# OthmanB/TAMCMC-C

Measured on AMD Instinct MI355X. Metric: MCMC samples/sec (whole node), 1e5 nu-bins x 100 params x 20 tempered chains, higher is better.
Workload: dtype f64

## Files before the change

include/tamcmc_sampler.h:

```cpp
#ifndef TAMCMC_SAMPLER_H
#define TAMCMC_SAMPLER_H

#include <stdint.h>

#include "tamcmc_hip.h"

#ifdef __cplusplus
extern "C" {
#endif

typedef struct tamcmc_sampler tamcmc_sampler;

typedef struct tamcmc_sampler_config {
    int32_t model_id;
    int32_t prior_class;
    int32_t likelihood_id;
    int32_t use_drift;
    double likelihood_params;
    int64_t Nparams;
    const double *inputs;
    const int32_t *relax;
    const int32_t *plength;
    const double *priors;
    const int32_t *priors_switch;
// ... 11 lines not shown
    double fd_step_rel;
    int32_t chain_groups;
    int32_t swap_rule;
} tamcmc_sampler_config;

int tamcmc_sampler_create(tamcmc_sampler **s, tamcmc_hip_ctx *ctx, const tamcmc_sampler_config *cfg);
void tamcmc_sampler_destroy(tamcmc_sampler *s);
int64_t tamcmc_sampler_nvars(const tamcmc_sampler *s);

#define TAMCMC_INFO_ENGINE 0
#define TAMCMC_INFO_NVARS 1
#define TAMCMC_INFO_NPARAMS 2
#define TAMCMC_INFO_NCHAINS 3
#define TAMCMC_INFO_ADAPT_IN_LDS 4
#define TAMCMC_INFO_FUSED_AVAILABLE 5
#define TAMCMC_INFO_CHAIN_GROUPS 6
#define TAMCMC_INFO_ITER_FUSED 7
#define TAMCMC_INFO_ITER_LOCKSTEP 8
#define TAMCMC_INFO_FUSED_STRETCHES 9
#define TAMCMC_INFO_QUICK_FALLBACKS 10
#define TAMCMC_INFO_QUICK_SURE 11
#define TAMCMC_INFO_ITER_JOINT 12
#define TAMCMC_INFO_ITER_WINDOW 13
#define TAMCMC_SAMPLER_INFO_N 14
int tamcmc_sampler_get_info(const tamcmc_sampler *s, int64_t *info, int32_t n);

int tamcmc_sampler_run(tamcmc_sampler *s, int64_t n_iter, double *samples, double *stats);
int tamcmc_sampler_run_packed(tamcmc_sampler *const *s, int32_t S, int64_t n_iter, double *const *samples, double *const *stats);

int tamcmc_sampler_draws(const tamcmc_sampler *s, int64_t iteration, double *z, double *u_accept, double *u_swap, int32_t *ind_A);

int tamcmc_sampler_get_state(const tamcmc_sampler *s, double *vars, double *logL, double *logPrior, double *logPost,
                             double *Pmove, double *sigma, int64_t *counters);
int tamcmc_sampler_get_gradient(const tamcmc_sampler *s, double *grad, double *grad_prior, int32_t *valid);
int tamcmc_sampler_get_last_test(const tamcmc_sampler *s, double *vars_prop, double *stats_prop, double *lq, double *grad_prop);
int tamcmc_sampler_get_tables(const tamcmc_sampler *s, int32_t *shape, void *rows, int32_t *nrows, double *noise, int32_t *nharvey,
                              int32_t *nnoise, int32_t *status, int32_t *written, double *logprior, double *params);
int tamcmc_sampler_get_move_counts(const tamcmc_sampler *s, int64_t *moves);
int tamcmc_sampler_get_proposal(const tamcmc_sampler *s, int32_t m, double *mu, double *covarmat);
int tamcmc_sampler_set_proposal(tamcmc_sampler *s, int32_t m, const double *mu, const double *covarmat, double sigma);
int tamcmc_sampler_seed_proposal_fisher(tamcmc_sampler *s, double hstep_rel, double *F );
int tamcmc_fisher_seed_covariance(int32_t Nvars, const double *F, const double *errors, double *cov);
int tamcmc_sampler_set_state(tamcmc_sampler *s, const double *vars, int64_t iteration);

int tamcmc_outputs_write_restore(const char *root, int32_t Nchains, int32_t Nvars, int64_t iteration, const char *const *names,
                                 const double *vars, const double *sigmas, const double *mus, const double *covarmats);
int tamcmc_outputs_read_restore(const char *root, int32_t *Nchains, int32_t *Nvars, int64_t *iteration, double *vars, double *sigmas,
// ... 29 lines not shown
```

tamcmc-c_amd/csrc/dev_sampler.h:

```cpp
#pragma once
#include <stdint.h>

#include "../../include/tamcmc_hip.h"
#if defined(__HIPCC__)
#include "dev_unpack.h"
#endif

#define TAMCMC_MAX_CHAINS 64

namespace tamcmc {

#if defined(__HIPCC__)
struct DevSamplerArgs {
    ModelDesc desc;
    int C, Nv, ntiles, chol_in_lds;
#ifdef TAMCMC_PROBE
    int probe = 0;
#endif
    int swap_rule;
    long pl;
    long dN_mixing;
    uint64_t seed;
    double c0, epsilon1, epsi2, A1, target_acceptance;
    const int *index_to_relax;
// ... 28 lines not shown
    int swap_rule = 0;
    int use_drift = 0;
    double delta = 0, fd_step_rel = 1e-7;
};

class DevSampler {
    struct Impl;
    Impl *impl;

  public:
    DevSampler();
    ~DevSampler();
    DevSampler(const DevSampler &) = delete;
    DevSampler &operator=(const DevSampler &) = delete;
    int init(tamcmc_hip_ctx *ctx, const DevSamplerInit &in);
    int upload_state(const double *vars, const double *params, const double *logL, const double *logPr,
                     const double *logPost, const double *init_logL);
    int upload_proposal(int m, const double *L_rowmajor, const double *cov, const double *mu, double sigma);
    int download_state(double *vars, double *params, double *logL, double *logPr, double *logPost, double *Pmove,
                       int *moved, long *counters, long *moves_per_chain = nullptr);
    int download_proposal(int m, double *cov, double *mu, double *sigma);
    int download_gradient(double *grad, double *grad_prior);
    int download_last_proposal(double *vars_prop, double *grad_prop);
    void info(long out[13]) const;
    int download_tables(int32_t shape[4], tamcmc_multiplet *rows, int32_t *nrows, double *noise, int32_t *nharvey, int32_t *nnoise,
                        int32_t *status, int32_t *written, double *logPr, double *params);
    int run(long it0, long n_iter, const char *learn, double *samples, double *stats);
    int run_mala(long it0, long n_iter, const char *learn, double *samples, double *stats);
};

}
```

tamcmc-c_amd/csrc/dev_sampler.hip:

```cpp
#include <hip/hip_runtime.h>

#include <atomic>
#include <chrono>
#include <hip/hip_ext.h>

#include <cmath>
#include <cstdio>
#include <cstdlib>
#include <cstring>
#include <algorithm>
#include <type_traits>
#include <utility>
#include <vector>

#include "ctx.h"
#include "rgb_prestep.h"
#include "rgb_front.h"
#include "dev_sampler.h"
#include "kernels.h"
#include "loglike_tile.h"
#include "dev_unpack.h"
#include "fd_batch.h"
#include "mode_tables.h"
#include "rng.h"
// ... 9 lines not shown

}


struct DevSampler::Impl {
    tamcmc_hip_ctx *ctx = nullptr;
    DevSamplerArgs a{};
    std::vector<void *> allocs;
    hipEvent_t ev[64][2];
    int n_ev = 0;
    bool poly_ready = false;
    double *adapt_scratch = nullptr;
    size_t smp_cap = 0, stat_cap = 0;
    size_t lds_base = 0, lds_adapt = 0;
    int parity = 0;
    FusedArgs f{};
    unsigned char *d_argcopy = nullptr;
    std::vector<unsigned char> h_argcopy;
    bool use_drift = false;
    double delta = 0, fd_step_rel = 1e-7;
    FdBatch fd;
    DevBuf<unsigned char> fd_block;
    DevBuf<double> fd_part, fd_S, fd_model, fd_bg;
    DevBuf<double> fused_bg, fused_part, fused_psum;
    MalaArgs mala{};
    bool grad_valid = false;
    int prior_class = 0, model_id = 0;
    std::vector<double> h_priors, h_extra;
    std::vector<int32_t> h_idx, h_sw;
    long armed_it = -1;
    int armed_q = 0;
    long it_fused = 0, it_lockstep = 0;
    long n_stretch = 0;
    long it_joint = 0, it_window = 0;
    int mala_chol_lds = -1;
    int last_scheme = 0, last_prop_parity = 0;

    hipEvent_t gev[8][2];
    int n_gev = 0;
    bool rgb = false;
    int rgb_bmax = 0;
    bool fused_ok = false;
    int fused_mode = -1, fused_K = 0;
    int tile_rot = 0;
    std::vector<int32_t> h_plength;
    int G = 1;
    hipStream_t gst[4] = {nullptr, nullptr, nullptr, nullptr};
// ... 44 lines not shown
        (void)hipStreamSynchronize(impl->ctx->stream);
        for (int g = 1; g < 4; g++) if (impl->gst[g]) (void)hipStreamSynchronize(impl->gst[g]);
    }
#ifdef TAMCMC_PROBE
    if (impl->a.counters && getenv("TAMCMC_PROBE_STEP")) {
        long h[40];
        (void)hipMemcpy(h, impl->a.counters + 8 + impl->a.C, sizeof h, hipMemcpyDeviceToHost);
        if (h[35] > 0) fprintf(stderr, "build_multiplet, row 20 (us): decode + widths/heights %.2f | window %.2f | m loop %.2f\n", 0.01 * h[32] / h[35], 0.01 * h[33] / h[35], 0.01 * h[34] / h[35]);
        for (int r = 0; r < 4; r++)
            if (h[8 * r + 3] > 0)
                fprintf(stderr, "candidate role %d of slot 2 (us): decide %.2f | vectors + L z %.2f | role %.2f  [inside: %.2f | %.2f]  (%ld launches)\n", r,
                        0.01 * h[8 * r] / h[8 * r + 3], 0.01 * h[8 * r + 1] / h[8 * r + 3], 0.01 * h[8 * r + 2] / h[8 * r + 3],
                        0.01 * h[8 * r + 4] / h[8 * r + 3], 0.01 * h[8 * r + 5] / h[8 * r + 3], h[8 * r + 3]);
    }
    if (impl->a.counters && getenv("TAMCMC_PROBE_ADAPT")) {
        long h[8];
        (void)hipMemcpy(h, impl->a.counters, sizeof h, hipMemcpyDeviceToHost);
        if (h[7] > 0)
            fprintf(stderr, "Cholesky panels of chain 0 (us per panel): columns below %.2f | next panel's columns %.2f | next diagonal block beside the rest of the trailing update %.2f  (%ld panels)\n",
                    0.01 * h[4] / h[7], 0.01 * h[5] / h[7], 0.01 * h[6] / h[7], h[7]);
    }
#endif
    for (void *p : impl->allocs) (void)hipFree(p);
    impl->fd_block.release(); impl->fd_part.release(); impl->fd_S.release(); impl->fd_model.release(); impl->fd_bg.release(); impl->fused_bg.release(); impl->fused_part.release(); impl->fused_psum.release();
    if (impl->h_pack) (void)hipHostFree(impl->h_pack);
    for (int i = 0; i < impl->n_ev; i++) { (void)hipEventDestroy(impl->ev[i][0]); (void)hipEventDestroy(impl->ev[i][1]); }
    for (int i = 0; i < impl->n_gev; i++) { (void)hipEventDestroy(impl->gev[i][0]); (void)hipEventDestroy(impl->gev[i][1]); }
    if (impl->ev_made) {
        (void)hipEventDestroy(impl->ev_fork);
        for (int g = 0; g < 4; g++) { (void)hipEventDestroy(impl->ev_kb[g]); (void)hipEventDestroy(impl->ev_ki[g]); (void)hipEventDestroy(impl->ev_join[g]); }
        for (int g = 1; g < 4; g++) if (impl->gst[g]) (void)hipStreamDestroy(impl->gst[g]);
    }
    delete impl;
}

#define DCHK(call)                                                                   \
    do {                                                                             \
        hipError_t e_ = (call);                                                      \
        if (e_ != hipSuccess) {                                                      \
            c->err = std::string(#call) + ": " + hipGetErrorString(e_);              \
            return TAMCMC_ERR_HIP;                                                   \
        }                                                                            \
    } while (0)

template <typename T>
static hipError_t up(T *dst, const T *src, size_t n, hipStream_t st) {
    return hipMemcpyAsync(dst, src, n * sizeof(T), hipMemcpyHostToDevice, st);
// ... 87 lines not shown
        I.gst[0] = st;
        for (int g = 1; g < G; g++) DCHK(hipStreamCreateWithFlags(&I.gst[g], hipStreamNonBlocking));
        DCHK(hipEventCreateWithFlags(&I.ev_fork, hipEventDisableTiming));
        for (int g = 0; g < 4; g++) {
            DCHK(hipEventCreateWithFlags(&I.ev_kb[g], hipEventDisableTiming));
            DCHK(hipEventCreateWithFlags(&I.ev_ki[g], hipEventDisableTiming));
            DCHK(hipEventCreateWithFlags(&I.ev_join[g], hipEventDisableTiming));
        }
        I.ev_made = true;
    }
    {
        FusedArgs &f = I.f;
        f.NS = 2 * in.C + 8;
        {
            const int h = (int)(((long)in.C * 1) / 2);
            f.xsplit = (I.G == 2 && h >= 3 && in.C - h >= 3) ? h : in.C;
        }
        const size_t NS = (size_t)f.NS;
        DCHK(I.dalloc(&f.cand_vars, 3 * NS * Nv)); DCHK(I.dalloc(&f.cand_params, 3 * NS * Np)); DCHK(I.dalloc(&f.cand_logPr, 6 * NS));
        DCHK(I.dalloc(&f.cand_stP, 6 * NS)); DCHK(I.dalloc(&f.cand_stR, 3 * NS)); DCHK(I.dalloc(&f.cand_rej, 3 * NS));
        DCHK(I.dalloc(&f.mults, 3 * NS * (size_t)a.desc.per + 1)); DCHK(I.dalloc(&f.pairs, 6 * NS)); DCHK(I.dalloc(&f.nh, 3 * NS)); DCHK(I.dalloc(&f.nn, 3 * NS));
        DCHK(I.dalloc(&f.noise, 3 * NS * (size_t)a.desc.stride));
        DCHK(I.dalloc(&f.slot, 2 * C)); DCHK(I.dalloc(&f.prop_logPr, 2 * C)); DCHK(I.dalloc(&f.prop_st, 2 * C)); DCHK(I.dalloc(&f.quick, 2 * C * QN)); DCHK(I.dalloc(&f.lz, 2 * C * Nv));
        DCHK(I.dalloc(&f.qcount, 2));
        DCHK(hipMemsetAsync(f.qcount, 0, 2 * sizeof(unsigned long long), st));
        f.qmargin = 1e-11;
        DCHK(hipMemsetAsync(f.nn, 0, 3 * NS * sizeof(int), st));
        DCHK(hipMemsetAsync(f.cand_stP, 0, 6 * NS * sizeof(int), st));
        DCHK(hipMemsetAsync(f.cand_rej, 0, 3 * NS * sizeof(int), st));
        DCHK(hipMemsetAsync(f.cand_stR, 0, 3 * NS * sizeof(int), st));
        f.part = nullptr;
        f.psum = nullptr;
        f.bg = nullptr;
        const size_t role_lds = (Np + 2 * Nv + 1) * sizeof(double) + unpack_lds_bytes() + 32;
        I.fused_ok = !I.rgb && role_lds <= sizeof(tile::TileLds<tile::M_FAST_DIRECT, 64>);
    }
    DCHK(hipStreamSynchronize(st));
    return TAMCMC_OK;
}

int DevSampler::download_gradient(double *grad, double *grad_prior) {
    Impl &I = *impl;
    tamcmc_hip_ctx *c = I.ctx;
    if (!I.use_drift || !I.a.grad_cur || !I.grad_valid) return TAMCMC_ERR_BAD_ARG;
    DCHK(hipSetDevice(c->device));
    const size_t n = (size_t)I.a.C * I.a.Nv;
    DCHK(hipStreamSynchronize(c->stream));
    if (grad) DCHK(hipMemcpy(grad, I.a.grad_cur + (size_t)I.parity * n, n * sizeof(double), hipMemcpyDeviceToHost));
    if (grad_prior) DCHK(hipMemcpy(grad_prior, I.a.gradP_cur + (size_t)I.parity * n, n * sizeof(double), hipMemcpyDeviceToHost));
    return TAMCMC_OK;
}

int DevSampler::download_last_proposal(double *vars_prop, double *grad_prop) {
    Impl &I = *impl;
    tamcmc_hip_ctx *c = I.ctx;
// ... 23 lines not shown
    std::vector<int32_t> pairs(2 * n), st(n), nn(n), rej(n, 0);
    std::vector<double> lp(fused ? 2 * n : n);
    auto get = [](void *dst, const void *src, size_t bytes) { return bytes ? hipMemcpy(dst, src, bytes, hipMemcpyDeviceToHost) : hipSuccess; };
    DCHK(get(pairs.data(), fused ? f.pairs : a.pairs, 2 * n * 4));
    DCHK(get(nn.data(), fused ? f.nn : a.nn, n * 4));
    DCHK(get(st.data(), fused ? f.cand_stR : a.status_prop + Q * C, n * 4));
    DCHK(get(lp.data(), fused ? f.cand_logPr : a.logPr_prop + Q * C, lp.size() * 8));
    if (fused) DCHK(get(rej.data(), f.cand_rej, n * 4));
    if (rows) DCHK(get(rows, fused ? f.mults : a.mults, n * per * sizeof(tamcmc_multiplet)));
    if (noise) DCHK(get(noise, fused ? f.noise : a.noise, n * stride * 8));
    if (nharvey) DCHK(get(nharvey, fused ? f.nh : a.nh, n * 4));
    if (params) DCHK(get(params, fused ? f.cand_params : a.params_prop + Q * C * Np, n * Np * 8));
    for (size_t s = 0; s < n; s++) {
        const bool w = !fused || nn[s] != 0 || st[s] != TAMCMC_OK;
        if (written) written[s] = w ? 1 : 0;
        if (nrows) nrows[s] = w ? pairs[2 * s + 1] - pairs[2 * s] : 0;
        if (nnoise) nnoise[s] = nn[s];
        if (status) status[s] = st[s];
        if (logPr) logPr[s] = fused ? (rej[s] ? -INFINITY : lp[2 * s] + lp[2 * s + 1]) : lp[s];
    }
    return TAMCMC_OK;
}

void DevSampler::info(long out[13]) const {
    const Impl &I = *impl;
    unsigned long long qc[2] = {0, 0};
    if (I.f.qcount && hipSetDevice(I.ctx->device) == hipSuccess) (void)hipMemcpy(qc, I.f.qcount, sizeof qc, hipMemcpyDeviceToHost);
    out[8] = I.n_stretch; out[9] = (long)qc[0]; out[10] = (long)qc[1];
    out[0] = I.a.Nv; out[1] = I.a.desc.Np;
    out[2] = I.use_drift ? I.mala_chol_lds : I.a.chol_in_lds;
    out[3] = (I.fused_ok && !I.use_drift) ? 1 : 0;
    out[4] = I.G; out[5] = I.it_fused; out[6] = I.it_lockstep; out[7] = I.a.C;
    out[11] = I.it_joint; out[12] = I.it_window;
}

int DevSampler::upload_state(const double *vars, const double *params, const double *logL, const double *logPr,
                             const double *logPost, const double *init_logL) {
    Impl &I = *impl;
    I.armed_it = -1;
    I.grad_valid = false;
    tamcmc_hip_ctx *c = I.ctx;
    DevSamplerArgs &a = I.a;
    const size_t C = (size_t)a.C, Np = (size_t)a.desc.Np, Nv = (size_t)a.Nv;
    hipStream_t st = c->stream;
    DCHK(hipSetDevice(c->device));
    const size_t P = (size_t)I.parity;
    DCHK(up(a.vars_cur + P * C * Nv, vars, C * Nv, st)); DCHK(up(a.params_cur + P * C * Np, params, C * Np, st));
    DCHK(up(a.logL_cur + P * C, logL, C, st)); DCHK(up(a.logPr_cur + P * C, logPr, C, st)); DCHK(up(a.logPost_cur + P * C, logPost, C, st));
    DCHK(up(a.init_logL, init_logL, C, st));
    DCHK(hipStreamSynchronize(st));
    {
// ... 226 lines not shown
    int prepare() {
        const size_t C = (size_t)a.C, Nv = (size_t)a.Nv;
        const int tb = tile_bins(c->wgs, c->K);
        a.ntiles = (a.desc.Nx + tb - 1) / tb;
        DCHK(c->d_part.reserve(C * (size_t)a.ntiles * 2));
        a.partials = c->d_part.p;
        a.tile_bins = tb;
        a.bg = nullptr;
        use_fused = I.fused_ok && c->step_scheme != 1 && c->wgs == 64 && (c->K == 4 || c->K == 8 || c->K == 16);
        I.f.qmargin = c->quick_decide == 1 ? (double)INFINITY : 1e-11;
        const size_t NS = (size_t)I.f.NS;
        I.f.bg = nullptr;
        if (c->precision == TAMCMC_PRECISION_FAST) {
            DCHK(c->d_bg.reserve(C * (size_t)a.ntiles * 8));
            a.bg = c->d_bg.p;
            if (use_fused) {
                DCHK(I.fused_bg.reserve(3 * NS * (size_t)a.ntiles * 8));
                I.f.bg = I.fused_bg.p;
            }
        }
        if (use_fused) {
            DCHK(I.fused_part.reserve(2 * C * (size_t)a.ntiles * 2));
            I.f.part = I.fused_part.p;
            DCHK(I.fused_psum.reserve(2 * C * (size_t)a.ntiles));
            I.f.psum = I.fused_psum.p;
        }
        split_ok = I.f.xsplit < a.C && c->step_scheme != 2 && (c->step_scheme == 3 || (long)a.C * a.ntiles >= 2500);
        auto grown = [](size_t need, size_t have, size_t unit) { const size_t floor_ = 256 * unit; return std::max(std::max(need, floor_), have * 2); };
        zc_smp = I.device_view(samples, (size_t)n_iter * C * Nv * 8);
        zc_st = I.device_view(stats, (size_t)n_iter * C * 3 * 8);
        if (samples && !zc_smp && I.smp_cap < (size_t)n_iter * C * Nv) {
            const size_t cap = grown((size_t)n_iter * C * Nv, I.smp_cap, C * Nv);
            DCHK(I.dalloc(&a.samples, cap));
            I.smp_cap = cap;
        }
        if (stats && !zc_st && I.stat_cap < (size_t)n_iter * C * 3) {
            const size_t cap = grown((size_t)n_iter * C * 3, I.stat_cap, C * 3);
            DCHK(I.dalloc(&a.stats, cap));
            I.stat_cap = cap;
        }
        args = a;
        args.samples = samples ? (zc_smp ? zc_smp : a.samples) : nullptr;
        args.stats = stats ? (zc_st ? zc_st : a.stats) : nullptr;
        const int G = I.G;
        for (int g = 0; g <= G; g++) goff[g] = (int)(((long)a.C * g) / G);
        auto fill_common = [&](LoglikeArgs &l, int B) {
            l.x = c->dx.p; l.y = c->dy.p; l.logx = c->dlogx.p; l.Nx = a.desc.Nx; l.B = B; l.ntiles = a.ntiles;
            l.x0 = a.desc.x_first; l.step = a.desc.step; l.noise_stride = a.desc.stride; l.model = nullptr; l.tile_rot = I.tile_rot;
// ... 390 lines not shown
```

tamcmc-c_amd/csrc/dev_step_impl.h:

```cpp

struct FusedArgs {
    int NS;
    int xsplit;
    double *cand_vars, *cand_params;
    double *cand_logPr;
    int *cand_rej;
    int *cand_stP, *cand_stR;
    tamcmc_multiplet *mults;
    int *pairs, *nh, *nn;
    double *noise;
    double *bg;
    int *slot;
    double *prop_logPr;
    int *prop_st;
    double *quick;
    double *part;
    double *psum;
    double *lz;
    double qmargin;
    unsigned long long *qcount;
};

constexpr int QN = 8;
constexpr int ST_L = 1, ST_BR = 2, ST_ENTRY = 4, ST_LZ = 8, ST_FIRST = 16, ST_COMMIT = 32;

typedef DevSamplerArgs __attribute__((address_space(4))) ConstArgs;
typedef FusedArgs __attribute__((address_space(4))) ConstFused;
__device__ __forceinline__ const void __attribute__((address_space(4))) *uniform_ptr(const void *p) {
    const unsigned long long v = (unsigned long long)p;
    const unsigned lo = (unsigned)__builtin_amdgcn_readfirstlane((int)(v & 0xffffffffull)), hi = (unsigned)__builtin_amdgcn_readfirstlane((int)(v >> 32));
    return (const void __attribute__((address_space(4))) *)(((unsigned long long)hi << 32) | lo);
}

struct Decided {
    int slot;
    int src;
    int src_acc;
    int src_par;
    int src_ps;
    int swap_first;
    int swapped;
    double r;
    AcceptOut o;
};

// ... 53 lines not shown
    if (!in_pair) {
        d.slot = 2 * m + o0.acc; d.src = m; d.src_acc = o0.acc; d.src_par = p; d.src_ps = ps0; d.r = o0.r; d.o = o0;
    } else {
        o1.acc = __shfl(o.acc, 1, 64); o1.r = __shfl(o.r, 1, 64); o1.logL = __shfl(o.logL, 1, 64); o1.logPr = __shfl(o.logPr, 1, 64);
        o1.logPost = __shfl(o.logPost, 1, 64);
        const int ps1 = __shfl(ps, 1, 64);
        const int accA = o0.acc, accB = o1.acc;
        const double rA = o0.r, rB = o1.r;
        const int swapped = resolve_swap(a, A, u, o0, o1);
        d.swap_first = A; d.swapped = swapped; d.src_par = p;
        const int B = A + 1;
        if (swapped) {
            if (m == A) { d.slot = 2 * C + (A >= f.xsplit ? 4 : 0) + accB; d.src = B; d.src_acc = accB; d.src_ps = ps1; d.r = rB; d.o = o0; }
            else { d.slot = 2 * C + (B >= f.xsplit ? 4 : 0) + 2 + accA; d.src = A; d.src_acc = accA; d.src_ps = ps0; d.r = rA; d.o = o1; }
        } else {
            if (m == A) { d.slot = 2 * A + accA; d.src = A; d.src_acc = accA; d.src_ps = ps0; d.r = rA; d.o = o0; }
            else { d.slot = 2 * B + accB; d.src = B; d.src_acc = accB; d.src_ps = ps1; d.r = rB; d.o = o1; }
        }
    }
    if (out && lane == 0) *out = d;
    return d.slot;
}

__device__ __attribute__((noinline)) void commit_chain(const DevSamplerArgs *ga, const FusedArgs *gf, int m, long it, int q, int settled, long rec,
                                                       int tiles, Decided *dec) {
    const int slot = decide(ga, gf, m, it, q, settled, dec);
    __syncthreads();
    const ConstArgs &a = *(const ConstArgs *)uniform_ptr(ga);
    const ConstFused &f = *(const ConstFused *)uniform_ptr(gf);
    const int lane = threadIdx.x, C = a.C, Nv = a.Nv, Np = a.desc.Np;
    const Decided d = *dec;
    if (lane == 0) {
        const size_t gs = (size_t)(it % 3) * f.NS + slot;
        const int stP0 = f.cand_stP[2 * gs], stP1 = f.cand_stP[2 * gs + 1], stR = f.cand_stR[gs];
        const double lp = f.cand_rej[gs] ? -INFINITY : f.cand_logPr[2 * gs] + f.cand_logPr[2 * gs + 1];
        const int stm = stP0 != TAMCMC_OK ? stP0 : (stP1 != TAMCMC_OK ? stP1 : stR);
        f.prop_logPr[q * C + m] = lp;
        f.prop_st[q * C + m] = stm;
        double *w = f.quick + ((size_t)q * C + m) * QN;
        const double Tm = a.Tcoefs[m];
        double Sstar = 0, ok = -1;
        double u, u1;
        rng_uniform2(a.seed, RNG_ACCEPT, (uint32_t)m, (uint64_t)it, 0, u, u1);
        if (stm == TAMCMC_OK && !(lp == -INFINITY || isnan(lp))) {
            const double cur = settled ? a.logPost_cur[q * C + m] : d.o.logPost;
            Sstar = -((log(u) - lp + cur) * Tm) / (double)a.pl;
            if (isfinite(Sstar)) ok = 1;
        } else if (u > 0.0) ok = 2;
        w[0] = Sstar; w[1] = ok; w[2] = -(double)a.pl / Tm; w[3] = settled ? a.logL_cur[q * C + m] : d.o.logL;
        double lus = 0, k1 = 0, k2 = 0;
// ... 23 lines not shown
    if (lane == 0) {
        a.logL_cur[q * C + m] = d.o.logL;
        a.logPr_cur[q * C + m] = d.o.logPr;
        a.logPost_cur[q * C + m] = d.o.logPost;
        f.slot[q * C + m] = slot;
        a.moved[m] = d.src_acc;
        a.Pmove[m] = d.r;
        if (m == 0 && d.src_acc) a.counters[1] += 1;
        a.counters[8 + m] += d.src_acc;
        if (m == 0) a.counters[0] = it;
        if (d.swap_first == m) {
            atomicAdd((unsigned long long *)&a.counters[2], 1ull);
            if (d.swapped) atomicAdd((unsigned long long *)&a.counters[3], 1ull);
        }
        if (a.stats && rec >= 0) {
            double *r = a.stats + ((size_t)rec * C + m) * 3;
            r[0] = d.o.logL; r[1] = d.o.logPr; r[2] = d.o.logPost;
        }
        if (tiles && d.swap_first < 0 && f.quick[((size_t)(q ^ 1) * C + m) * QN + 1] == 2.0) atomicAdd(f.qcount + 1, 1ull);
    }
}


template <bool PAIR>
__device__ __forceinline__ void quick_sums(const double *c0, int n, int lane, double &s0, double &a0, double &s1, double &a1) {
    for (int t0 = 0; t0 < n; t0 += 256) {
        double v[4], w[4];
#pragma unroll
        for (int k = 0; k < 4; k++) {
            const int t = t0 + k * 64 + lane;
            v[k] = t < n ? c0[t] : 0.0;
            if (PAIR) w[k] = t < n ? c0[n + t] : 0.0;
        }
#pragma unroll
        for (int k = 0; k < 4; k++) {
            s0 += v[k]; a0 += fabs(v[k]);
            if (PAIR) { s1 += w[k]; a1 += fabs(w[k]); }
        }
    }
#pragma unroll
    for (int off = 32; off >= 1; off >>= 1) {
        s0 += __shfl_xor(s0, off, 64); a0 += __shfl_xor(a0, off, 64);
        if (PAIR) { s1 += __shfl_xor(s1, off, 64); a1 += __shfl_xor(a1, off, 64); }
    }
}
__device__ __forceinline__ int quick_decide_core(const DevSamplerArgs *ga, const FusedArgs *gf, int m, int q, int pairA, Decided *out) {
    const ConstArgs &a = *(const ConstArgs *)uniform_ptr(ga);
    const ConstFused &f = *(const ConstFused *)uniform_ptr(gf);
    const int lane = threadIdx.x & 63, C = a.C;
    const int p = q ^ 1, n = a.ntiles;
    const bool in_pair = pairA >= 0 && (m == pairA || m == pairA + 1);
    const int j0 = in_pair ? pairA : m;
    const double *c0 = f.psum + ((size_t)p * C + j0) * n;
    const double *r0 = f.quick + ((size_t)p * C + j0) * QN;
    double rec, s0 = 0, a0 = 0, s1 = 0, a1 = 0;
    if (in_pair) {
        rec = lane < 2 * QN ? r0[lane] : 0.0;
        quick_sums<true>(c0, n, lane, s0, a0, s1, a1);
    } else {
        rec = lane < QN ? r0[lane] : 0.0;
        quick_sums<false>(c0, n, lane, s0, a0, s1, a1);
    }
    const double St0 = __shfl(rec, 0, 64), ok0 = __shfl(rec, 1, 64);
    const int ps0 = (int)__shfl(rec, 7, 64);
    const double mg = f.qmargin;
    int acc0 = 0;
    if (ok0 == 2.0) { s0 = 0; a0 = 0; }
    else if (ok0 > 0 && fabs(s0 - St0) > mg * (a0 + fabs(St0))) acc0 = s0 < St0 ? 1 : 0;
    else return -1;
    Decided d;
    d.swap_first = -1; d.swapped = 0; d.src_par = p; d.r = 0;
    d.o.acc = 0; d.o.r = 0; d.o.logL = 0; d.o.logPr = 0; d.o.logPost = 0;
    if (!in_pair) { d.slot = 2 * m + acc0; d.src = m; d.src_acc = acc0; d.src_ps = ps0; }
    else {
        const double St1 = __shfl(rec, QN, 64), ok1 = __shfl(rec, QN + 1, 64);
        const int ps1 = (int)__shfl(rec, QN + 7, 64);
        int acc1 = 0;
        if (ok1 == 2.0) { s1 = 0; a1 = 0; }
        else if (ok1 > 0 && fabs(s1 - St1) > mg * (a1 + fabs(St1))) acc1 = s1 < St1 ? 1 : 0;
        else return -1;
        const double c0 = __shfl(rec, 2, 64), c1 = __shfl(rec, QN + 2, 64);
        const double LA = acc0 ? c0 * s0 : __shfl(rec, 3, 64), LB = acc1 ? c1 * s1 : __shfl(rec, QN + 3, 64);
        const double lus = __shfl(rec, 4, 64), x = LA * __shfl(rec, 5, 64) + LB * __shfl(rec, 6, 64);
        if (!(fabs(x - lus) > mg * (fabs(c0) * a0 + fabs(c1) * a1 + fabs(LA) + fabs(LB)))) return -1;
        const int swapped = x > lus ? 1 : 0;
        const int A = pairA, B = pairA + 1;
        d.swap_first = A; d.swapped = swapped;
        if (swapped) {
            if (m == A) { d.slot = 2 * C + (A >= f.xsplit ? 4 : 0) + acc1; d.src = B; d.src_acc = acc1; d.src_ps = ps1; }
            else { d.slot = 2 * C + (B >= f.xsplit ? 4 : 0) + 2 + acc0; d.src = A; d.src_acc = acc0; d.src_ps = ps0; }
        } else {
            if (m == A) { d.slot = 2 * A + acc0; d.src = A; d.src_acc = acc0; d.src_ps = ps0; }
            else { d.slot = 2 * B + acc1; d.src = B; d.src_acc = acc1; d.src_ps = ps1; }
        }
    }
    if (out && lane == 0) *out = d;
    return d.slot;
}
__device__ __attribute__((noinline)) int quick_decide_leaf(const DevSamplerArgs *ga, const FusedArgs *gf, int m, int q, int pairA, Decided *out) {
    return quick_decide_core(ga, gf, m, q, pairA, out);
}

__device__ __forceinline__ int quick_decide(const DevSamplerArgs *ga, const FusedArgs *gf, int m, long it, int q, int settled, int pairA,
                                            Decided *out) {
    if (settled) return decide(ga, gf, m, it, q, 1, out);
    const int s = quick_decide_leaf(ga, gf, m, q, pairA, out);
    return s >= 0 ? s : decide(ga, gf, m, it, q, 0, out);
}

__device__ __attribute__((noinline)) int decide_counted(const DevSamplerArgs *ga, const FusedArgs *gf, int m, long it, int q, int tile) {
    if (tile == 0 && (threadIdx.x & 63) == 0) atomicAdd(((const ConstFused *)uniform_ptr(gf))->qcount, 1ull);
    return decide(ga, gf, m, it, q, 0, nullptr);
}

struct StepTiles {
    const DevSamplerArgs *ga;
    const FusedArgs *gf;
    long it;
    int q, first, settled, pairA;
    static constexpr bool early_loads = true;
    __device__ __forceinline__ tile::SlotWords head(const LoglikeArgs &a, int b, int tile) const {
        const int m = first + b;
        if (settled) return tile::slot_words(a, decide(ga, gf, m, it, q, 1, nullptr));
        const bool lone = a.per > 0 && !(pairA >= 0 && (m == pairA || m == pairA + 1));
        tile::SlotWords w0{}, w1{};
        if (lone) { w0 = tile::slot_words(a, 2 * m); w1 = tile::slot_words(a, 2 * m + 1); }
        int s = quick_decide_core(ga, gf, m, q, pairA, nullptr);
        if (s < 0) s = decide_counted(ga, gf, m, it, q, tile);
        if (lone && (s >> 1) == m) return (s & 1) ? w1 : w0;
        return tile::slot_words(a, s);
    }
    __device__ __forceinline__ void store_sums(int b, int tile, double s0, double s1) const {
        const ConstArgs &a = *(const ConstArgs *)uniform_ptr(ga);
        const ConstFused &f = *(const ConstFused *)uniform_ptr(gf);
        f.psum[((size_t)q * a.C + first + b) * a.ntiles + tile] = s0 + s1;
    }
};

__device__ __attribute__((noinline)) void role_prior(const DevSamplerArgs *ga, const FusedArgs *gf, size_t gs, int h, const double *s_vars,
                                                     const double *s_params, const UnpackLds *Up) {
    const DevSamplerArgs &a = *ga;
    const FusedArgs &f = *gf;
    const UnpackLds U = *Up;
    const int Nv = a.Nv, Np = a.desc.Np, tid = threadIdx.x;
    if (h == 0) {
        for (int i = tid; i < Nv; i += 64) f.cand_vars[gs * Nv + i] = s_vars[i];
        for (int i = tid; i < Np; i += 64) f.cand_params[gs * Np + i] = s_params[i];
    }
    int rej = 0;
#ifdef TAMCMC_PROBE
    long ps_[4] = {0, 0, 0, 0};
    const double fh = wave_log_prior_part(a.desc, s_params, U, TB - 128, h, &rej, ps_);
    if (tid == 0 && (int)(gs % f.NS) == 2) { long *w = a.counters + 8 + a.C + 16 * h + 4; w[0] += ps_[1] - ps_[0]; w[1] += ps_[2] - ps_[1]; }
#else
    const double fh = wave_log_prior_part(a.desc, s_params, U, TB - 128, h, &rej);
#endif
    if (tid == 0) {
        f.cand_logPr[2 * gs + h] = fh;
// ... 230 lines not shown
```

tamcmc-c_amd/csrc/host_capi.cpp:

```cpp
#include <cmath>
#include <cstring>
#include <memory>
#include <vector>
#include <string>
#include <thread>

#include "../../include/tamcmc_sampler.h"
#include "dev_sampler.h"
#include "host_sampler.h"
#include "rng.h"
#include "step_schedule.h"

using namespace tamcmc;

extern "C" {
void tamcmc_hip_ctx_attach(tamcmc_hip_ctx *c);
void tamcmc_hip_ctx_detach(tamcmc_hip_ctx *c);
}

struct tamcmc_sampler {
    Config cfg;
    std::unique_ptr<MALA> mala;
    std::unique_ptr<Model_def> cur, prop;
    std::unique_ptr<DevSampler> dev;
// ... 120 lines not shown
    s->attached = true;
    *out = s.release();
    return TAMCMC_OK;
}

void tamcmc_sampler_destroy(tamcmc_sampler *s) {
    if (!s) return;
    tamcmc_hip_ctx *ctx = s->attached ? s->ctx : nullptr;
    delete s;
    tamcmc_hip_ctx_detach(ctx);
}

int64_t tamcmc_sampler_nvars(const tamcmc_sampler *s) { return s ? s->cur->get_Nvars() : -1; }

int tamcmc_sampler_get_info(const tamcmc_sampler *s, int64_t *info, int32_t n) {
    if (!s || !info || n < 1) return TAMCMC_ERR_BAD_ARG;
    int64_t v[TAMCMC_SAMPLER_INFO_N] = {0};
    v[TAMCMC_INFO_ENGINE] = s->dev ? 1 : 0;
    v[TAMCMC_INFO_NVARS] = s->cur->get_Nvars();
    v[TAMCMC_INFO_NPARAMS] = s->cur->get_Nparams();
    v[TAMCMC_INFO_NCHAINS] = s->cfg.MALA.Nchains;
    v[TAMCMC_INFO_ADAPT_IN_LDS] = -1;
    if (s->dev) {
        long d[13];
        s->dev->info(d);
        v[TAMCMC_INFO_ADAPT_IN_LDS] = d[2];
        v[TAMCMC_INFO_FUSED_AVAILABLE] = d[3];
        v[TAMCMC_INFO_CHAIN_GROUPS] = d[4];
        v[TAMCMC_INFO_ITER_FUSED] = d[5];
        v[TAMCMC_INFO_ITER_LOCKSTEP] = d[6];
        v[TAMCMC_INFO_FUSED_STRETCHES] = d[8];
        v[TAMCMC_INFO_QUICK_FALLBACKS] = d[9];
        v[TAMCMC_INFO_QUICK_SURE] = d[10];
        v[TAMCMC_INFO_ITER_JOINT] = d[11];
        v[TAMCMC_INFO_ITER_WINDOW] = d[12];
    }
    for (int32_t i = 0; i < n && i < TAMCMC_SAMPLER_INFO_N; i++) info[i] = v[i];
    return TAMCMC_OK;
}

int tamcmc_sampler_run(tamcmc_sampler *s, int64_t n_iter, double *samples, double *stats) {
    if (!s || n_iter < 0) return TAMCMC_ERR_BAD_ARG;
    const long Nc = s->cfg.MALA.Nchains, Nv = s->cur->get_Nvars();
    if (s->dev) {
        const long it0 = s->mala->iteration;
        std::vector<char> learn((size_t)n_iter);
        bool any = false;
        for (int64_t i = 0; i < n_iter; i++) { learn[(size_t)i] = s->mala->learn_at(it0 + i) ? 1 : 0; any = any || learn[(size_t)i]; }
// ... 320 lines not shown
```

tamcmc-c_amd/sampler.py:

```python
import ctypes as C

import numpy as np

from . import ABI, EXTRA_ABI, HipContext, TamcmcError, OK, lib, _dp, _ip, _vp, _f64, _i32, _p

_i64p = C.POINTER(C.c_int64)


class SamplerConfig(C.Structure):
    _fields_ = [("model_id", C.c_int32), ("prior_class", C.c_int32), ("likelihood_id", C.c_int32), ("use_drift", C.c_int32),
                ("likelihood_params", C.c_double), ("Nparams", C.c_int64), ("inputs", _dp), ("relax", _ip), ("plength", _ip),
                ("priors", _dp), ("priors_switch", _ip), ("extra_priors", _dp), ("n_extra", C.c_int32),
                ("Nchains", C.c_int32), ("lambda_temp", C.c_double), ("target_acceptance", C.c_double), ("c0", C.c_double),
                ("epsilon1", C.c_double), ("epsilon2", C.c_double), ("A1", C.c_double), ("delta", C.c_double),
                ("delta_x", C.c_double), ("Nt_learn", _i64p), ("periods_learn", _i64p), ("n_Nt_learn", C.c_int32),
                ("engine", C.c_int32), ("dN_mixing", C.c_int64), ("init_errors", _dp), ("seed", C.c_uint64),
                ("fd_step_rel", C.c_double), ("chain_groups", C.c_int32), ("swap_rule", C.c_int32)]


EXTRA_ABI += [
    ("tamcmc_sampler_create", C.c_int, [C.POINTER(_vp), _vp, C.POINTER(SamplerConfig)]),
    ("tamcmc_sampler_destroy", None, [_vp]),
    ("tamcmc_sampler_nvars", C.c_int64, [_vp]),
    ("tamcmc_sampler_get_info", C.c_int, [_vp, _i64p, C.c_int32]),
# ... 98 lines not shown
            record, stats = smp is not None, stt is not None
            for arr, shape, what in ((smp, (n_iter, self.nchains, self.nvars), "samples"), (stt, (n_iter, self.nchains, 3), "stats")):
                if arr is not None and not (isinstance(arr, np.ndarray) and arr.flags.c_contiguous and arr.dtype == np.float64 and arr.shape == shape):
                    raise ValueError(f"out: {what} must be a C-contiguous float64 array of shape {shape}")
        else:
            smp = np.zeros((n_iter, self.nchains, self.nvars)) if record else None
            stt = np.zeros((n_iter, self.nchains, 3)) if stats else None
        st = self._L.tamcmc_sampler_run(self._h, n_iter, _p(smp), _p(stt))
        if st != OK:
            raise TamcmcError(st, self._L.tamcmc_hip_last_error(self.ctx._h).decode())
        return smp, stt

    def state(self):
        nc, nv = self.nchains, self.nvars
        out = {"vars": np.zeros((nc, nv)), "logL": np.zeros(nc), "logPrior": np.zeros(nc), "logPost": np.zeros(nc),
               "Pmove": np.zeros(nc), "sigma": np.zeros(nc)}
        cnt = np.zeros(4, dtype=np.int64)
        self._L.tamcmc_sampler_get_state(self._h, _p(out["vars"]), _p(out["logL"]), _p(out["logPrior"]), _p(out["logPost"]),
                                         _p(out["Pmove"]), _p(out["sigma"]), _p(cnt, _i64p))
        out.update(iteration=int(cnt[0]), accepted0=int(cnt[1]), swap_attempts=int(cnt[2]), swaps=int(cnt[3]))
        return out

    def info(self):
        v = np.zeros(14, dtype=np.int64)
        rc = self._L.tamcmc_sampler_get_info(self._h, _p(v, _i64p), 14)
        if rc != OK:
            raise TamcmcError(rc, "tamcmc_sampler_get_info")
        keys = ("engine", "nvars", "nparams", "nchains", "adapt_in_lds", "fused_available", "chain_groups", "iter_fused", "iter_lockstep",
                "fused_stretches", "quick_fallbacks", "quick_sure", "iter_joint", "iter_window")
        return dict(zip(keys, (int(x) for x in v)))

    def gradient(self):
        g, gp = np.zeros((self.nchains, self.nvars)), np.zeros((self.nchains, self.nvars))
        v = np.zeros(self.nchains, dtype=np.int32)
        rc = self._L.tamcmc_sampler_get_gradient(self._h, _p(g), _p(gp), _p(v, _ip))
        if rc != OK:
            raise TamcmcError(rc, "tamcmc_sampler_get_gradient")
        return g, gp, v

    def last_test(self):
        v, st, lq = np.zeros((self.nchains, self.nvars)), np.zeros((self.nchains, 3)), np.zeros((self.nchains, 2))
        g = np.zeros((self.nchains, self.nvars))
        rc = self._L.tamcmc_sampler_get_last_test(self._h, _p(v), _p(st), _p(lq), _p(g))
        if rc != OK:
            raise TamcmcError(rc, "tamcmc_sampler_get_last_test")
        return v, st, lq, g

    def tables(self):
        from . import MULT_DTYPE
        shape = np.zeros(4, dtype=np.int32)
        rc = self._L.tamcmc_sampler_get_tables(self._h, _p(shape, _ip), None, None, None, None, None, None, None, None, None)
        if rc != OK:
# ... 198 lines not shown
```

Baseline: 50180.

## Accumulate quick-decide partial sums via atomics into per-chain lines instead of per-tile arrays

```diff
diff --git a/include/tamcmc_sampler.h b/include/tamcmc_sampler.h
--- a/include/tamcmc_sampler.h
+++ b/include/tamcmc_sampler.h
@@ -57,7 +57,8 @@
 #define TAMCMC_INFO_QUICK_SURE 11
 #define TAMCMC_INFO_ITER_JOINT 12
 #define TAMCMC_INFO_ITER_WINDOW 13
-#define TAMCMC_SAMPLER_INFO_N 14
+#define TAMCMC_INFO_QUICK_MISMATCH 14
+#define TAMCMC_SAMPLER_INFO_N 15
 int tamcmc_sampler_get_info(const tamcmc_sampler *s, int64_t *info, int32_t n);
 
 int tamcmc_sampler_run(tamcmc_sampler *s, int64_t n_iter, double *samples, double *stats);
diff --git a/tamcmc-c_amd/csrc/dev_sampler.h b/tamcmc-c_amd/csrc/dev_sampler.h
--- a/tamcmc-c_amd/csrc/dev_sampler.h
+++ b/tamcmc-c_amd/csrc/dev_sampler.h
@@ -74,7 +74,7 @@
     int download_proposal(int m, double *cov, double *mu, double *sigma);
     int download_gradient(double *grad, double *grad_prior);
     int download_last_proposal(double *vars_prop, double *grad_prop);
-    void info(long out[13]) const;
+    void info(long out[14]) const;
     int download_tables(int32_t shape[4], tamcmc_multiplet *rows, int32_t *nrows, double *noise, int32_t *nharvey, int32_t *nnoise,
                         int32_t *status, int32_t *written, double *logPr, double *params);
     int run(long it0, long n_iter, const char *learn, double *samples, double *stats);
diff --git a/tamcmc-c_amd/csrc/dev_sampler.hip b/tamcmc-c_amd/csrc/dev_sampler.hip
--- a/tamcmc-c_amd/csrc/dev_sampler.hip
+++ b/tamcmc-c_amd/csrc/dev_sampler.hip
@@ -55,7 +55,7 @@
     FdBatch fd;
     DevBuf<unsigned char> fd_block;
     DevBuf<double> fd_part, fd_S, fd_model, fd_bg;
-    DevBuf<double> fused_bg, fused_part, fused_psum;
+    DevBuf<double> fused_bg, fused_part;
     MalaArgs mala{};
     bool grad_valid = false;
     int prior_class = 0, model_id = 0;
@@ -146,7 +146,7 @@
     }
 #endif
     for (void *p : impl->allocs) (void)hipFree(p);
-    impl->fd_block.release(); impl->fd_part.release(); impl->fd_S.release(); impl->fd_model.release(); impl->fd_bg.release(); impl->fused_bg.release(); impl->fused_part.release(); impl->fused_psum.release();
+    impl->fd_block.release(); impl->fd_part.release(); impl->fd_S.release(); impl->fd_model.release(); impl->fd_bg.release(); impl->fused_bg.release(); impl->fused_part.release();
     if (impl->h_pack) (void)hipHostFree(impl->h_pack);
     for (int i = 0; i < impl->n_ev; i++) { (void)hipEventDestroy(impl->ev[i][0]); (void)hipEventDestroy(impl->ev[i][1]); }
     for (int i = 0; i < impl->n_gev; i++) { (void)hipEventDestroy(impl->gev[i][0]); (void)hipEventDestroy(impl->gev[i][1]); }
@@ -280,15 +280,18 @@
         DCHK(I.dalloc(&f.mults, 3 * NS * (size_t)a.desc.per + 1)); DCHK(I.dalloc(&f.pairs, 6 * NS)); DCHK(I.dalloc(&f.nh, 3 * NS)); DCHK(I.dalloc(&f.nn, 3 * NS));
         DCHK(I.dalloc(&f.noise, 3 * NS * (size_t)a.desc.stride));
         DCHK(I.dalloc(&f.slot, 2 * C)); DCHK(I.dalloc(&f.prop_logPr, 2 * C)); DCHK(I.dalloc(&f.prop_st, 2 * C)); DCHK(I.dalloc(&f.quick, 2 * C * QN)); DCHK(I.dalloc(&f.lz, 2 * C * Nv));
-        DCHK(I.dalloc(&f.qcount, 2));
-        DCHK(hipMemsetAsync(f.qcount, 0, 2 * sizeof(unsigned long long), st));
+        DCHK(I.dalloc(&f.qcount, 3));
+        DCHK(hipMemsetAsync(f.qcount, 0, 3 * sizeof(unsigned long long), st));
+        static_assert(2 * QK * sizeof(double) == 128, "one line per (set, chain)");
+        DCHK(I.dalloc(&f.qacc, 3 * C * 2 * QK));
+        if (((uintptr_t)f.qacc & 127) != 0) return TAMCMC_ERR_HIP;
+        DCHK(hipMemset(f.qacc, 0, 3 * C * 2 * QK * sizeof(double)));
         f.qmargin = 1e-11;
         DCHK(hipMemsetAsync(f.nn, 0, 3 * NS * sizeof(int), st));
         DCHK(hipMemsetAsync(f.cand_stP, 0, 6 * NS * sizeof(int), st));
         DCHK(hipMemsetAsync(f.cand_rej, 0, 3 * NS * sizeof(int), st));
         DCHK(hipMemsetAsync(f.cand_stR, 0, 3 * NS * sizeof(int), st));
         f.part = nullptr;
-        f.psum = nullptr;
         f.bg = nullptr;
         const size_t role_lds = (Np + 2 * Nv + 1) * sizeof(double) + unpack_lds_bytes() + 32;
         I.fused_ok = !I.rgb && role_lds <= sizeof(tile::TileLds<tile::M_FAST_DIRECT, 64>);
@@ -358,11 +361,11 @@
     return TAMCMC_OK;
 }
 
-void DevSampler::info(long out[13]) const {
+void DevSampler::info(long out[14]) const {
     const Impl &I = *impl;
-    unsigned long long qc[2] = {0, 0};
+    unsigned long long qc[3] = {0, 0, 0};
     if (I.f.qcount && hipSetDevice(I.ctx->device) == hipSuccess) (void)hipMemcpy(qc, I.f.qcount, sizeof qc, hipMemcpyDeviceToHost);
-    out[8] = I.n_stretch; out[9] = (long)qc[0]; out[10] = (long)qc[1];
+    out[8] = I.n_stretch; out[9] = (long)qc[0]; out[10] = (long)qc[1]; out[13] = (long)qc[2];
     out[0] = I.a.Nv; out[1] = I.a.desc.Np;
     out[2] = I.use_drift ? I.mala_chol_lds : I.a.chol_in_lds;
     out[3] = (I.fused_ok && !I.use_drift) ? 1 : 0;
@@ -635,8 +638,6 @@
         if (use_fused) {
             DCHK(I.fused_part.reserve(2 * C * (size_t)a.ntiles * 2));
             I.f.part = I.fused_part.p;
-            DCHK(I.fused_psum.reserve(2 * C * (size_t)a.ntiles));
-            I.f.psum = I.fused_psum.p;
         }
         split_ok = I.f.xsplit < a.C && c->step_scheme != 2 && (c->step_scheme == 3 || (long)a.C * a.ntiles >= 2500);
         auto grown = [](size_t need, size_t have, size_t unit) { const size_t floor_ = 256 * unit; return std::max(std::max(need, floor_), have * 2); };
diff --git a/tamcmc-c_amd/csrc/dev_step_impl.h b/tamcmc-c_amd/csrc/dev_step_impl.h
--- a/tamcmc-c_amd/csrc/dev_step_impl.h
+++ b/tamcmc-c_amd/csrc/dev_step_impl.h
@@ -15,12 +15,13 @@
     int *prop_st;
     double *quick;
     double *part;
-    double *psum;
     double *lz;
+    double *qacc;
     double qmargin;
     unsigned long long *qcount;
 };
 
+constexpr int QK = 8;
 constexpr int QN = 8;
 constexpr int ST_L = 1, ST_BR = 2, ST_ENTRY = 4, ST_LZ = 8, ST_FIRST = 16, ST_COMMIT = 32;
 
@@ -120,10 +121,35 @@
     return d.slot;
 }
 
+__device__ int quick_decide_leaf(const DevSamplerArgs *ga, const FusedArgs *gf, int m, int q, int es, int pairA, Decided *out);
+__device__ __attribute__((noinline)) void commit_sums(const DevSamplerArgs *ga, const FusedArgs *gf, int m, long it, int q, int settled, int tiles,
+                                                      int slot, int swap_first) {
+    const ConstArgs &a = *(const ConstArgs *)uniform_ptr(ga);
+    const ConstFused &f = *(const ConstFused *)uniform_ptr(gf);
+    const int lane = threadIdx.x, C = a.C;
+    const int pairA = settled ? -1 : __builtin_amdgcn_readfirstlane(swap_first);
+    const bool second = !tiles && pairA >= 0 && pairA != m;
+    int differs = 0;
+    if (!settled && !second) {
+        const int es = (int)((it + 2) % 3);
+        const int qs = quick_decide_leaf(ga, gf, m, q, es, pairA, nullptr);
+        differs = (qs >= 0 && qs != slot) ? 1 : 0;
+        if (lane == 0 && differs) atomicAdd(f.qcount + 2, 1ull);
+    }
+    const int z = lane;
+    if (tiles) {
+        if (z < 2 * QK) f.qacc[((size_t)((it + 1) % 3) * C + m) * (2 * QK) + z] = 0.0;
+    } else if (!second && z < 3 * 2 * QK) {
+        const size_t e = (size_t)(z / (2 * QK)) * C + m;
+        f.qacc[e * (2 * QK) + z % (2 * QK)] = 0.0;
+        if (pairA == m) f.qacc[(e + 1) * (2 * QK) + z % (2 * QK)] = 0.0;
+    }
+}
 __device__ __attribute__((noinline)) void commit_chain(const DevSamplerArgs *ga, const FusedArgs *gf, int m, long it, int q, int settled, long rec,
                                                        int tiles, Decided *dec) {
     const int slot = decide(ga, gf, m, it, q, settled, dec);
     __syncthreads();
+    commit_sums(ga, gf, m, it, q, settled, tiles, slot, dec->swap_first);
     const ConstArgs &a = *(const ConstArgs *)uniform_ptr(ga);
     const ConstFused &f = *(const ConstFused *)uniform_ptr(gf);
     const int lane = threadIdx.x, C = a.C, Nv = a.Nv, Np = a.desc.Np;
@@ -193,47 +219,32 @@
 }
 
 
-template <bool PAIR>
-__device__ __forceinline__ void quick_sums(const double *c0, int n, int lane, double &s0, double &a0, double &s1, double &a1) {
-    for (int t0 = 0; t0 < n; t0 += 256) {
-        double v[4], w[4];
-#pragma unroll
-        for (int k = 0; k < 4; k++) {
-            const int t = t0 + k * 64 + lane;
-            v[k] = t < n ? c0[t] : 0.0;
-            if (PAIR) w[k] = t < n ? c0[n + t] : 0.0;
-        }
-#pragma unroll
-        for (int k = 0; k < 4; k++) {
-            s0 += v[k]; a0 += fabs(v[k]);
-            if (PAIR) { s1 += w[k]; a1 += fabs(w[k]); }
-        }
-    }
-#pragma unroll
-    for (int off = 32; off >= 1; off >>= 1) {
-        s0 += __shfl_xor(s0, off, 64); a0 += __shfl_xor(a0, off, 64);
-        if (PAIR) { s1 += __shfl_xor(s1, off, 64); a1 += __shfl_xor(a1, off, 64); }
-    }
-}
-__device__ __forceinline__ int quick_decide_core(const DevSamplerArgs *ga, const FusedArgs *gf, int m, int q, int pairA, Decided *out) {
+__device__ __forceinline__ double row_sum_by_parity(double x) {
+#define TAMCMC_ROW_ROR(x, n)                                                                                                     \
+    __longlong_as_double(((long long)__builtin_amdgcn_update_dpp(0, (int)(__double_as_longlong(x) >> 32), 0x120 + (n), 0xf, 0xf, false) << 32) | \
+                         (unsigned int)__builtin_amdgcn_update_dpp(0, (int)(__double_as_longlong(x) & 0xffffffffll), 0x120 + (n), 0xf, 0xf, false))
+    x += TAMCMC_ROW_ROR(x, 8);
+    x += TAMCMC_ROW_ROR(x, 4);
+    x += TAMCMC_ROW_ROR(x, 2);
+#undef TAMCMC_ROW_ROR
+    return x;
+}
+
+__device__ __forceinline__ int quick_decide_core(const DevSamplerArgs *ga, const FusedArgs *gf, int m, int q, int es, int pairA, Decided *out) {
     const ConstArgs &a = *(const ConstArgs *)uniform_ptr(ga);
     const ConstFused &f = *(const ConstFused *)uniform_ptr(gf);
     const int lane = threadIdx.x & 63, C = a.C;
-    const int p = q ^ 1, n = a.ntiles;
+    const int p = q ^ 1;
     const bool in_pair = pairA >= 0 && (m == pairA || m == pairA + 1);
     const int j0 = in_pair ? pairA : m;
-    const double *c0 = f.psum + ((size_t)p * C + j0) * n;
     const double *r0 = f.quick + ((size_t)p * C + j0) * QN;
-    double rec, s0 = 0, a0 = 0, s1 = 0, a1 = 0;
-    if (in_pair) {
-        rec = lane < 2 * QN ? r0[lane] : 0.0;
-        quick_sums<true>(c0, n, lane, s0, a0, s1, a1);
-    } else {
-        rec = lane < QN ? r0[lane] : 0.0;
-        quick_sums<false>(c0, n, lane, s0, a0, s1, a1);
-    }
-    const double St0 = __shfl(rec, 0, 64), ok0 = __shfl(rec, 1, 64);
-    const int ps0 = (int)__shfl(rec, 7, 64);
+    const double *g0 = f.qacc + ((size_t)es * C + j0) * (2 * QK);
+    const double rec = lane < (in_pair ? 2 * QN : QN) ? r0[lane] : 0.0;
+    const double acc = lane < (in_pair ? 4 * QK : 2 * QK) ? g0[lane] : 0.0;
+    const double sums = row_sum_by_parity(acc);
+    double s0 = lane_value<0>(sums), a0 = lane_value<1>(sums);
+    const double St0 = lane_value<0>(rec), ok0 = lane_value<1>(rec);
+    const int ps0 = (int)lane_value<7>(rec);
     const double mg = f.qmargin;
     int acc0 = 0;
     if (ok0 == 2.0) { s0 = 0; a0 = 0; }
@@ -244,15 +255,16 @@
     d.o.acc = 0; d.o.r = 0; d.o.logL = 0; d.o.logPr = 0; d.o.logPost = 0;
     if (!in_pair) { d.slot = 2 * m + acc0; d.src = m; d.src_acc = acc0; d.src_ps = ps0; }
     else {
-        const double St1 = __shfl(rec, QN, 64), ok1 = __shfl(rec, QN + 1, 64);
-        const int ps1 = (int)__shfl(rec, QN + 7, 64);
+        double s1 = lane_value<16>(sums), a1 = lane_value<17>(sums);
+        const double St1 = lane_value<QN>(rec), ok1 = lane_value<QN + 1>(rec);
+        const int ps1 = (int)lane_value<QN + 7>(rec);
         int acc1 = 0;
         if (ok1 == 2.0) { s1 = 0; a1 = 0; }
         else if (ok1 > 0 && fabs(s1 - St1) > mg * (a1 + fabs(St1))) acc1 = s1 < St1 ? 1 : 0;
         else return -1;
-        const double c0 = __shfl(rec, 2, 64), c1 = __shfl(rec, QN + 2, 64);
-        const double LA = acc0 ? c0 * s0 : __shfl(rec, 3, 64), LB = acc1 ? c1 * s1 : __shfl(rec, QN + 3, 64);
-        const double lus = __shfl(rec, 4, 64), x = LA * __shfl(rec, 5, 64) + LB * __shfl(rec, 6, 64);
+        const double c0 = lane_value<2>(rec), c1 = lane_value<QN + 2>(rec);
+        const double LA = acc0 ? c0 * s0 : lane_value<3>(rec), LB = acc1 ? c1 * s1 : lane_value<QN + 3>(rec);
+        const double lus = lane_value<4>(rec), x = LA * lane_value<5>(rec) + LB * lane_value<6>(rec);
         if (!(fabs(x - lus) > mg * (fabs(c0) * a0 + fabs(c1) * a1 + fabs(LA) + fabs(LB)))) return -1;
         const int swapped = x > lus ? 1 : 0;
         const int A = pairA, B = pairA + 1;
@@ -268,14 +280,14 @@
     if (out && lane == 0) *out = d;
     return d.slot;
 }
-__device__ __attribute__((noinline)) int quick_decide_leaf(const DevSamplerArgs *ga, const FusedArgs *gf, int m, int q, int pairA, Decided *out) {
-    return quick_decide_core(ga, gf, m, q, pairA, out);
+__device__ __attribute__((noinline)) int quick_decide_leaf(const DevSamplerArgs *ga, const FusedArgs *gf, int m, int q, int es, int pairA, Decided *out) {
+    return quick_decide_core(ga, gf, m, q, es, pairA, out);
 }
 
 __device__ __forceinline__ int quick_decide(const DevSamplerArgs *ga, const FusedArgs *gf, int m, long it, int q, int settled, int pairA,
                                             Decided *out) {
     if (settled) return decide(ga, gf, m, it, q, 1, out);
-    const int s = quick_decide_leaf(ga, gf, m, q, pairA, out);
+    const int s = quick_decide_leaf(ga, gf, m, q, (int)((it + 2) % 3), pairA, out);
     return s >= 0 ? s : decide(ga, gf, m, it, q, 0, out);
 }
 
@@ -296,15 +308,18 @@
         const bool lone = a.per > 0 && !(pairA >= 0 && (m == pairA || m == pairA + 1));
         tile::SlotWords w0{}, w1{};
         if (lone) { w0 = tile::slot_words(a, 2 * m); w1 = tile::slot_words(a, 2 * m + 1); }
-        int s = quick_decide_core(ga, gf, m, q, pairA, nullptr);
+        int s = quick_decide_core(ga, gf, m, q, (int)((it + 2) % 3), pairA, nullptr);
         if (s < 0) s = decide_counted(ga, gf, m, it, q, tile);
         if (lone && (s >> 1) == m) return (s & 1) ? w1 : w0;
         return tile::slot_words(a, s);
     }
-    __device__ __forceinline__ void store_sums(int b, int tile, double s0, double s1) const {
+    __device__ __forceinline__ void store_sums(int b, int , double s0, double s1) const {
         const ConstArgs &a = *(const ConstArgs *)uniform_ptr(ga);
         const ConstFused &f = *(const ConstFused *)uniform_ptr(gf);
-        f.psum[((size_t)q * a.C + first + b) * a.ntiles + tile] = s0 + s1;
+        const double c = s0 + s1;
+        double *g = f.qacc + (((size_t)(it % 3) * a.C + first + b) * QK + (blockIdx.x & 7)) * 2;
+        atomicAdd(g, c);
+        atomicAdd(g + 1, fabs(c));
     }
 };
 
diff --git a/tamcmc-c_amd/csrc/host_capi.cpp b/tamcmc-c_amd/csrc/host_capi.cpp
--- a/tamcmc-c_amd/csrc/host_capi.cpp
+++ b/tamcmc-c_amd/csrc/host_capi.cpp
@@ -166,8 +166,9 @@
     v[TAMCMC_INFO_NCHAINS] = s->cfg.MALA.Nchains;
     v[TAMCMC_INFO_ADAPT_IN_LDS] = -1;
     if (s->dev) {
-        long d[13];
+        long d[14];
         s->dev->info(d);
+        v[TAMCMC_INFO_QUICK_MISMATCH] = d[13];
         v[TAMCMC_INFO_ADAPT_IN_LDS] = d[2];
         v[TAMCMC_INFO_FUSED_AVAILABLE] = d[3];
         v[TAMCMC_INFO_CHAIN_GROUPS] = d[4];
diff --git a/tamcmc-c_amd/sampler.py b/tamcmc-c_amd/sampler.py
--- a/tamcmc-c_amd/sampler.py
+++ b/tamcmc-c_amd/sampler.py
@@ -144,12 +144,12 @@
         return out
 
     def info(self):
-        v = np.zeros(14, dtype=np.int64)
-        rc = self._L.tamcmc_sampler_get_info(self._h, _p(v, _i64p), 14)
+        v = np.zeros(15, dtype=np.int64)
+        rc = self._L.tamcmc_sampler_get_info(self._h, _p(v, _i64p), 15)
         if rc != OK:
             raise TamcmcError(rc, "tamcmc_sampler_get_info")
         keys = ("engine", "nvars", "nparams", "nchains", "adapt_in_lds", "fused_available", "chain_groups", "iter_fused", "iter_lockstep",
-                "fused_stretches", "quick_fallbacks", "quick_sure", "iter_joint", "iter_window")
+                "fused_stretches", "quick_fallbacks", "quick_sure", "iter_joint", "iter_window", "quick_mismatch")
         return dict(zip(keys, (int(x) for x in v)))
 
     def gradient(self):
```

Result: faster. 50740, median of 6 (+1.1%).
